# zkonduit/ezkl

Hardware: NVIDIA H100
Metric: prove_time_s (lower is better)
Workload: dtype u32 limbs (254-bit Montgomery integers mod BN254 r/p)

## Files before the change

### ezkl_b200/csrc/capi.cu

```cuda
#include <atomic>
#include <cerrno>
#include <condition_variable>
#include <cstdlib>
#include <cstring>
#include <deque>
#include <functional>
#include <mutex>
#include <string>
#include <thread>
#include <unordered_map>
#include <vector>

#include "../../include/ezkl_b200.h"
#include "msm.cuh"
#include "ntt.cuh"
#include "poly.cuh"
#include "quotient.cuh"

namespace b200 {

static Config g_cfg;
const Config& config() { return g_cfg; }
int sm_count() {
    static std::atomic<int> cache[64];
    int dev = 0;
    if (cudaGetDevice(&dev) != cudaSuccess || dev < 0 || dev >= 64) return 132;
    int v = cache[dev].load(std::memory_order_relaxed);
    if (v == 0) {
        if (cudaDeviceGetAttribute(&v, cudaDevAttrMultiProcessorCount, dev) != cudaSuccess || v <= 0) v = 132;
        cache[dev].store(v, std::memory_order_relaxed);
    }
    return v;
}
static int env_int(const char* name, int dflt) { const char* e = getenv(name); return e ? atoi(e) : dflt; }
static int read_config() {
    Config c;
    if (const char* e = getenv("B200_MSM_TABLE_MB")) {
        char* end = nullptr;
        errno = 0;
        const unsigned long long mb = strtoull(e, &end, 10);
        B200_CHECK(*e >= '0' && *e <= '9' && *end == '\0' && errno == 0 && mb >= 1 && mb < ((unsigned long long)1 << 40), -1,
                   "b200_init: B200_MSM_TABLE_MB = '%s' is not a positive whole number of MiB", e);
        c.msm_table_budget = (size_t)mb << 20;
    }
    if (const char* e = getenv("B200_WS_BUDGET_MB")) c.ws_budget_call = (size_t)atol(e) << 20;
    if (const char* e = getenv("B200_WS_TOTAL_MB")) c.ws_budget_total = (size_t)atol(e) << 20;
    c.msm_reduce_m = env_int("B200_MSM_REDUCE_M", 0);
    c.msm_reduce_threads = env_int("B200_MSM_REDUCE_THREADS", 0);
    c.shard_min_logn = env_int("B200_SHARD_MIN_LOGN", 22);
    g_cfg = c;
    return 0;
}

static constexpr int MAX_DEV = 8;
struct DeviceState { int id = -1; NttContext ntt; };
static DeviceState g_devs[MAX_DEV];
static std::atomic<int> g_ndev{0};
static std::atomic<bool> g_inited{false};
static std::atomic<int> g_active{0};
static std::atomic<uint64_t> g_epoch{1};
static std::mutex g_mu;

struct BaseSet {
    size_t n = 0; int c = 0, W = 0, s = 1, L = 0;
    MsmTable* t[MAX_DEV] = {};
};
static std::unordered_map<uint64_t, BaseSet*> g_tables;
static uint64_t g_next_handle = 1;

struct Ctx {
    int slot = 0, dev = 0;
    cudaStream_t stream = nullptr;
    MsmWorkspace msm_ws;
    PolyWorkspace poly_ws;
    QuotientWorkspace quot_ws;
    StagingRing ring;
    DevBuf stage_a, stage_b, stage_c, small;
    uint8_t* bounce[2] = {nullptr, nullptr};
    cudaEvent_t bounce_ev[2] = {nullptr, nullptr};
    cudaEvent_t last_ev = nullptr;
    cudaStream_t last_stream = nullptr;
    bool has_last = false;
    void release() {
        cudaSetDevice(dev);
        DevBuf* bufs[] = {&msm_ws.counts, &msm_ws.offs, &msm_ws.ents, &msm_ws.subs, &msm_ws.sums, &msm_ws.misc, &poly_ws.scratch, &quot_ws.prog,
                          &stage_a, &stage_b, &stage_c, &small};
        for (DevBuf* b : bufs) b->release();
        ring.release(); poly_ws.ring.release(); quot_ws.ring.release();
        for (int i = 0; i < 2; ++i) { if (bounce[i]) cudaFreeHost(bounce[i]); if (bounce_ev[i]) cudaEventDestroy(bounce_ev[i]); bounce[i] = nullptr; bounce_ev[i] = nullptr; }
        if (last_ev) cudaEventDestroy(last_ev);
        if (stream) cudaStreamDestroy(stream);
        last_ev = nullptr; stream = nullptr;
    }
};
static std::vector<Ctx*> g_ctxs;
static std::atomic<int> g_nctx{0};

struct TlCtx {
    Ctx* c[MAX_DEV] = {};
    uint64_t epoch = 0;
    ~TlCtx() {
        if (epoch != g_epoch.load() || !g_inited.load()) return;
        std::lock_guard<std::mutex> lk(g_mu);
        if (epoch != g_epoch.load()) return;
        int cur = 0; cudaGetDevice(&cur);
        for (int s = 0; s < MAX_DEV; ++s) if (c[s]) {
            for (size_t i = 0; i < g_ctxs.size(); ++i) if (g_ctxs[i] == c[s]) { g_ctxs.erase(g_ctxs.begin() + i); break; }
            c[s]->release(); delete c[s]; g_nctx--;
        }
        cudaSetDevice(cur);
    }
};
static thread_local TlCtx tl;

struct CallGuard {
    bool ok;
    CallGuard() { g_active++; ok = g_inited.load(); if (!ok) set_error("b200: not initialised (call b200_init first)"); }
    ~CallGuard() { g_active--; }
};

static int get_ctx(Ctx** out, int slot = 0) {
    if (!g_inited.load()) { set_error("b200: not initialised (call b200_init first)"); return -3; }
    const uint64_t ep = g_epoch.load();
    if (tl.epoch != ep) { for (int s = 0; s < MAX_DEV; ++s) tl.c[s] = nullptr; tl.epoch = ep; }
    B200_CHECK(slot >= 0 && slot < g_ndev.load(), -1, "b200: device slot %d out of range", slot);
    if (!tl.c[slot]) {
        Ctx* c = new Ctx();
        c->slot = slot; c->dev = g_devs[slot].id;
        int cur = 0; cudaGetDevice(&cur);
        cudaError_t e = cudaSetDevice(c->dev);
        if (e == cudaSuccess) e = cudaStreamCreateWithFlags(&c->stream, cudaStreamNonBlocking);
        if (e == cudaSuccess) e = cudaEventCreateWithFlags(&c->last_ev, cudaEventDisableTiming);
        if (g_ndev.load() > 1) cudaSetDevice(cur);
        if (e != cudaSuccess) { set_error("b200: context creation on device %d failed: %s", c->dev, cudaGetErrorString(e)); delete c; return -2; }
        std::lock_guard<std::mutex> lk(g_mu);
        g_ctxs.push_back(c); g_nctx++;
        tl.c[slot] = c;
    }
    *out = tl.c[slot];
    return 0;
}
static int slot_of(const void* dptr) {
    const int nd = g_ndev.load();
    if (nd <= 1 || !dptr) return 0;
    cudaPointerAttributes at;
    if (cudaPointerGetAttributes(&at, dptr) != cudaSuccess) { cudaGetLastError(); return 0; }
    for (int s = 0; s < nd; ++s) if (g_devs[s].id == at.device) return s;
    return 0;
}
struct DevGuard {
    int prev = -1;
    explicit DevGuard(const Ctx* c) { if (g_ndev.load() > 1) { cudaGetDevice(&prev); if (prev != c->dev) cudaSetDevice(c->dev); else prev = -1; } }
    ~DevGuard() { if (prev >= 0) cudaSetDevice(prev); }
};
struct StreamScope {
    Ctx* c; cudaStream_t st;
    StreamScope(Ctx* c_, void* user) : c(c_), st(user ? (cudaStream_t)user : c_->stream) {
        if (c->has_last && c->last_stream != st) cudaStreamWaitEvent(st, c->last_ev, 0);
    }
    ~StreamScope() { if (cudaEventRecord(c->last_ev, st) == cudaSuccess) { c->last_stream = st; c->has_last = true; } else cudaGetLastError(); }
};
#define B200_ENTER(c, dptr)                                                \
    CallGuard _cg; if (!_cg.ok) return -3;                                 \
    Ctx* c; if (int _rc = get_ctx(&c, slot_of(dptr))) return _rc;          \
    DevGuard _dg(c)

static size_t call_budget() {
    if (g_cfg.ws_budget_call) return g_cfg.ws_budget_call;
// ... 1090 lines not shown
```

### ezkl_b200/csrc/debug.cu

```cuda
#include "../../include/ezkl_b200.h"
#include "msm.cuh"
#include "ntt.cuh"

namespace b200 {
template <class Tag>
__global__ void k_dbg_field(int op, const Fp<Tag>* a, const Fp<Tag>* b, Fp<Tag>* o, size_t n) {
    size_t i = (size_t)blockIdx.x * blockDim.x + threadIdx.x;
    if (i >= n) return;
    Fp<Tag> x = fp_load(a + i), y = fp_load(b + i), r;
    if (op == 0) r = x + y; else if (op == 1) r = x - y; else if (op == 2) r = x * y; else if (op == 3) r = fp_inv(x); else r = fp_from_mont(x);
    fp_store(o + i, r);
}
__global__ void k_dbg_g1(int op, const G1Affine* a, const G1Affine* b, G1Affine* o, size_t n) {
    size_t i = (size_t)blockIdx.x * blockDim.x + threadIdx.x;
    if (i >= n) return;
    G1Affine p = a[i], q = b[i];
    G1Xyzz r;
    if (op == 0) r = g1_add_mixed(g1_to_xyzz(p), q);
    else if (op == 1) r = g1_dbl(g1_to_xyzz(p));
    else if (op == 2) r = g1_mul_small(g1_to_xyzz(p), q.x.l[0]);
    else if (op == 3) r = g1_add(g1_to_xyzz(p), g1_dbl_affine(q));
    else r = g1_add_mixed(g1_to_xyzz(p), g1_neg(p));
    o[i] = g1_to_affine(r);
}
__global__ void k_dbg_digits(const Fr* s, int c, int W, int32_t* out, size_t n) {
    size_t i = (size_t)blockIdx.x * blockDim.x + threadIdx.x;
    if (i >= n) return;
    Fr v = fp_from_mont(fp_load(s + i));
    uint32_t carry = 0;
    for (int w = 0; w < W; ++w) out[i * W + w] = msm_next_digit(v.l, c, &carry);
}
template <int VARIANT>
__global__ void __launch_bounds__(256) k_bench_mul(Fq* out, int iters) {
    const uint32_t t = blockIdx.x * blockDim.x + threadIdx.x;
    Fq x = fp_one<FqTag>(), y = fp_one<FqTag>();
    x.l[0] ^= t; y.l[1] ^= (t * 2654435761u);
    if (VARIANT == 0) {
#pragma unroll 1
        for (int i = 0; i < iters; ++i) x = x * y;
    } else if (VARIANT == 1) {
        Fq z = y + y;
#pragma unroll 1
        for (int i = 0; i < iters; i += 2) { x = x * y; z = z * y; }
        x = x + z;
    } else if (VARIANT == 2) {
#pragma unroll 1
        for (int i = 0; i < iters; ++i) { Fq r; fp_mul_portable<FqTag>(r.l, x.l, y.l); x = r; }
    } else if (VARIANT == 3) {
        G1Affine g; g.x = x; g.y = y;
        G1Xyzz acc = g1_dbl_affine(g);
#pragma unroll 1
        for (int i = 0; i < iters; ++i) { acc = g1_add_mixed(acc, g); g.x.l[0] += 1; }
        x = acc.x + acc.y + acc.zz + acc.zzz;
    } else {
#pragma unroll 1
        for (int i = 0; i < iters; ++i) { x = x + y; y = y - x; }
    }
    fp_store(out + t, x);
}
template <int V>
__global__ void __launch_bounds__(256) k_bench_pipe(uint64_t* out, int iters) {
    const uint32_t t = blockIdx.x * blockDim.x + threadIdx.x;
    uint32_t a = t * 2654435761u + 12345u, b = t ^ 0x9e3779b9u;
    if (V == 0) {
        uint64_t c0 = t, c1 = t + 1, c2 = t + 2, c3 = t + 3, c4 = t + 4, c5 = t + 5, c6 = t + 6, c7 = t + 7;
#pragma unroll 1
        for (int i = 0; i < iters; ++i) {
            asm volatile("mad.wide.u32 %0, %8, %9, %0;\n\tmad.wide.u32 %1, %8, %9, %1;\n\tmad.wide.u32 %2, %8, %9, %2;\n\tmad.wide.u32 %3, %8, %9, %3;\n\t"
                         "mad.wide.u32 %4, %8, %9, %4;\n\tmad.wide.u32 %5, %8, %9, %5;\n\tmad.wide.u32 %6, %8, %9, %6;\n\tmad.wide.u32 %7, %8, %9, %7;"
                         : "+l"(c0), "+l"(c1), "+l"(c2), "+l"(c3), "+l"(c4), "+l"(c5), "+l"(c6), "+l"(c7) : "r"(a), "r"(b));
        }
        out[t] = c0 ^ c1 ^ c2 ^ c3 ^ c4 ^ c5 ^ c6 ^ c7;
    } else if (V == 1) {
        uint32_t e0 = t, e1 = 1, e2 = 2, e3 = 3, e4 = 4, e5 = 5, e6 = 6, e7 = 7, o0 = 8, o1 = 9, o2 = 10, o3 = 11, o4 = 12, o5 = 13, o6 = 14, o7 = 15;
#pragma unroll 1
        for (int i = 0; i < iters; ++i) {
            asm volatile("mad.lo.cc.u32 %0, %16, %17, %0;\n\tmadc.hi.cc.u32 %1, %16, %17, %1;\n\tmadc.lo.cc.u32 %2, %16, %17, %2;\n\tmadc.hi.cc.u32 %3, %16, %17, %3;\n\t"
                         "madc.lo.cc.u32 %4, %16, %17, %4;\n\tmadc.hi.cc.u32 %5, %16, %17, %5;\n\tmadc.lo.cc.u32 %6, %16, %17, %6;\n\tmadc.hi.u32 %7, %16, %17, %7;\n\t"
                         "mad.lo.cc.u32 %8, %16, %17, %8;\n\tmadc.hi.cc.u32 %9, %16, %17, %9;\n\tmadc.lo.cc.u32 %10, %16, %17, %10;\n\tmadc.hi.cc.u32 %11, %16, %17, %11;\n\t"
                         "madc.lo.cc.u32 %12, %16, %17, %12;\n\tmadc.hi.cc.u32 %13, %16, %17, %13;\n\tmadc.lo.cc.u32 %14, %16, %17, %14;\n\tmadc.hi.u32 %15, %16, %17, %15;"
                         : "+r"(e0), "+r"(e1), "+r"(e2), "+r"(e3), "+r"(e4), "+r"(e5), "+r"(e6), "+r"(e7), "+r"(o0), "+r"(o1), "+r"(o2), "+r"(o3), "+r"(o4), "+r"(o5), "+r"(o6), "+r"(o7)
                         : "r"(a), "r"(b));
        }
        out[t] = (uint64_t)(e0 ^ e1 ^ e2 ^ e3 ^ e4 ^ e5 ^ e6 ^ e7) << 32 | (o0 ^ o1 ^ o2 ^ o3 ^ o4 ^ o5 ^ o6 ^ o7);
    } else if (V == 2) {
        uint32_t c0 = t, c1 = 1, c2 = 2, c3 = 3, c4 = 4, c5 = 5, c6 = 6, c7 = 7;
#pragma unroll 1
        for (int i = 0; i < iters; ++i) {
            asm volatile("mad.lo.u32 %0, %8, %9, %0;\n\tmad.lo.u32 %1, %8, %9, %1;\n\tmad.lo.u32 %2, %8, %9, %2;\n\tmad.lo.u32 %3, %8, %9, %3;\n\t"
                         "mad.lo.u32 %4, %8, %9, %4;\n\tmad.lo.u32 %5, %8, %9, %5;\n\tmad.lo.u32 %6, %8, %9, %6;\n\tmad.lo.u32 %7, %8, %9, %7;"
                         : "+r"(c0), "+r"(c1), "+r"(c2), "+r"(c3), "+r"(c4), "+r"(c5), "+r"(c6), "+r"(c7) : "r"(a), "r"(b));
        }
        out[t] = c0 ^ c1 ^ c2 ^ c3 ^ c4 ^ c5 ^ c6 ^ c7;
    } else {
        double x = (double)a, y = 1.0 + 1e-9 * (double)(b & 1023), c0 = t, c1 = 1, c2 = 2, c3 = 3, c4 = 4, c5 = 5, c6 = 6, c7 = 7;
#pragma unroll 1
        for (int i = 0; i < iters; ++i) {
            c0 = fma(x, y, c0); c1 = fma(x, y, c1); c2 = fma(x, y, c2); c3 = fma(x, y, c3); c4 = fma(x, y, c4); c5 = fma(x, y, c5); c6 = fma(x, y, c6); c7 = fma(x, y, c7);
        }
        out[t] = (uint64_t)(c0 + c1 + c2 + c3 + c4 + c5 + c6 + c7);
    }
}
}
using namespace b200;

#pragma GCC visibility push(default)
extern "C" {
// ... 16 lines not shown
    B200_CUDA(cudaGetLastError());
    B200_CUDA(cudaMemcpy(out, dout, 64 * n, cudaMemcpyDeviceToHost));
    cudaFree(da); cudaFree(db); cudaFree(dout);
    return 0;
}
int b200_debug_digits(const b200_fr* s, size_t n, int c, int32_t* out ) {
    const int W = (255 + c - 1) / c;
    void *ds, *dout;
    B200_CUDA(cudaMalloc(&ds, 32 * n)); B200_CUDA(cudaMalloc(&dout, 4 * n * W));
    B200_CUDA(cudaMemcpy(ds, s, 32 * n, cudaMemcpyHostToDevice));
    k_dbg_digits<<<div_up(n, 128), 128>>>((const Fr*)ds, c, W, (int32_t*)dout, n);
    B200_CUDA(cudaGetLastError());
    B200_CUDA(cudaMemcpy(out, dout, 4 * n * W, cudaMemcpyDeviceToHost));
    cudaFree(ds); cudaFree(dout);
    return 0;
}
int b200_debug_bench(int variant, int iters, int blocks, int threads, float* ms) {
    Fq* d; B200_CUDA(cudaMalloc(&d, sizeof(Fq) * (size_t)blocks * threads));
    cudaEvent_t e0, e1; cudaEventCreate(&e0); cudaEventCreate(&e1);
    for (int rep = 0; rep < 2; ++rep) {
        cudaEventRecord(e0);
        switch (variant) {
            case 0: k_bench_mul<0><<<blocks, threads>>>(d, iters); break;
            case 1: k_bench_mul<1><<<blocks, threads>>>(d, iters); break;
            case 2: k_bench_mul<2><<<blocks, threads>>>(d, iters); break;
            case 3: k_bench_mul<3><<<blocks, threads>>>(d, iters); break;
            default: k_bench_mul<4><<<blocks, threads>>>(d, iters); break;
        }
        cudaEventRecord(e1);
        B200_CUDA(cudaEventSynchronize(e1));
    }
    B200_CUDA(cudaEventElapsedTime(ms, e0, e1));
    cudaFree(d); cudaEventDestroy(e0); cudaEventDestroy(e1);
    return 0;
}
int b200_debug_bench_pipe(int variant, int iters, int blocks, int threads, float* ms) {
    uint64_t* d; B200_CUDA(cudaMalloc(&d, 8 * (size_t)blocks * threads));
    cudaEvent_t e0, e1; cudaEventCreate(&e0); cudaEventCreate(&e1);
    for (int rep = 0; rep < 2; ++rep) {
        cudaEventRecord(e0);
        switch (variant) {
            case 0: k_bench_pipe<0><<<blocks, threads>>>(d, iters); break;
            case 1: k_bench_pipe<1><<<blocks, threads>>>(d, iters); break;
            case 2: k_bench_pipe<2><<<blocks, threads>>>(d, iters); break;
            default: k_bench_pipe<3><<<blocks, threads>>>(d, iters); break;
        }
        cudaEventRecord(e1);
        B200_CUDA(cudaEventSynchronize(e1));
    }
    B200_CUDA(cudaEventElapsedTime(ms, e0, e1));
    cudaFree(d); cudaEventDestroy(e0); cudaEventDestroy(e1);
    return 0;
}
int b200_debug_digits_host(const b200_fr* s_canonical, size_t n, int c, int32_t* out) {
    const int W = (255 + c - 1) / c;
    for (size_t i = 0; i < n; ++i) {
        uint32_t v[8]; memcpy(v, &s_canonical[i], 32);
        uint32_t carry = 0;
        for (int w = 0; w < W; ++w) out[i * W + w] = msm_next_digit(v, c, &carry);
    }
    return 0;
}
int b200_debug_digit_slots_host(const b200_fr* s_canonical, size_t n, int c, int wpl, int32_t* out) {
    const int W = (255 + c - 1) / c;
    for (size_t i = 0; i < n; ++i) {
        uint32_t v[8]; memcpy(v, &s_canonical[i], 32);
        uint32_t carry = 0;
        MsmWindowSlot slot;
        for (int w = 0; w < W; ++w) {
            const int32_t d = msm_next_digit(v, c, &carry);
            int32_t* o = out + ((size_t)i * W + w) * 4;
            o[0] = (int32_t)slot.level; o[1] = slot.r;
            o[2] = d ? (int32_t)(slot.set_off + (uint32_t)(d < 0 ? -d : d) - 1u) : -1;
            o[3] = d < 0 ? -1 : (d > 0 ? 1 : 0);
            slot.next(c, wpl);
        }
    }
    return 0;
}
int b200_debug_msm_pick_levels(size_t n, int c, size_t max_table_bytes, int* s, int* L) {
    msm_pick_levels(n, c, max_table_bytes, s, L);
    return 0;
}
int b200_debug_ntt_plan_host(uint32_t log_n, int batch, int sm_count, int64_t* out ) {
    if (log_n < 1 || log_n > 28 || batch < 1 || batch > 65535 || sm_count < 1) return -1;
    int npass, logm[3];
    ntt_choose_passes(log_n, &npass, logm);
    for (int i = 0; i < npass; ++i) {
        const NttPassShape sh = ntt_pass_shape(npass, logm, i);
        const NttPassGeom g = ntt_pass_geometry((uint32_t)logm[i], sh.inner_cnt, sh.lines, batch, sm_count);
        int64_t* o = out + 7 * i;
        o[0] = g.kernel; o[1] = logm[i]; o[2] = g.log_g; o[3] = g.threads; o[4] = (int64_t)g.smem; o[5] = (int64_t)g.grid_x;
        o[6] = i == npass - 1 ? 0 : (g.kernel == 2 && ntt_full_table(log_n, npass) ? 1 : 2);
    }
    return npass;
}
int b200_debug_host_g1_op(int op, const b200_g1_affine* a, const b200_g1_affine* b, b200_g1_affine* out, size_t n) {
    for (size_t i = 0; i < n; ++i) {
        G1Affine p, q; memcpy(&p, &a[i], 64); memcpy(&q, &b[i], 64);
        G1Xyzz r;
        if (op == 0) r = g1_add_mixed(g1_to_xyzz(p), q);
        else if (op == 1) r = g1_dbl(g1_to_xyzz(p));
        else if (op == 2) r = g1_mul_small(g1_to_xyzz(p), q.x.l[0]);
        else if (op == 3) r = g1_add(g1_to_xyzz(p), g1_dbl_affine(q));
        else r = g1_add_mixed(g1_to_xyzz(p), g1_neg(p));
        G1Affine o = g1_to_affine(r); memcpy(&out[i], &o, 64);
    }
    return 0;
}
int b200_debug_host_field_op(int field, int op, const b200_fr* a, const b200_fr* b, b200_fr* out, size_t n) {
    for (size_t i = 0; i < n; ++i) {
        if (field == 0) { Fr x, y, r; memcpy(&x, &a[i], 32); memcpy(&y, &b[i], 32);
            if (op == 0) r = x + y; else if (op == 1) r = x - y; else if (op == 2) r = x * y; else if (op == 3) r = fp_inv(x); else r = fp_from_mont(x);
            memcpy(&out[i], &r, 32);
        } else { Fq x, y, r; memcpy(&x, &a[i], 32); memcpy(&y, &b[i], 32);
            if (op == 0) r = x + y; else if (op == 1) r = x - y; else if (op == 2) r = x * y; else if (op == 3) r = fp_inv(x); else r = fp_from_mont(x);
            memcpy(&out[i], &r, 32);
        }
    }
    return 0;
}
}
#pragma GCC visibility pop
```

### ezkl_b200/csrc/msm.cu

```cuda
#include "msm.cuh"
#include "ec_coop.cuh"

namespace b200 {

static constexpr int HEAVY_CHUNKS = 32;
static constexpr int REDUCE_M_MAX = 32;
static constexpr int TREE_THREADS = 256;

int msm_default_window(size_t n) {
    int k = 0;
    while (((size_t)1 << (k + 1)) <= n) ++k;
    int c = k <= 10 ? 8 : (k <= 13 ? k - 2 : (k <= 17 ? k - 1 : (k <= 19 ? 17 : (k <= 21 ? 18 : 20))));
    if (c < 4) c = 4;
    if (c > 22) c = 22;
    return c;
}

__global__ void __launch_bounds__(128) k_table_next_level(const G1Affine* __restrict__ prev, G1Affine* __restrict__ next, size_t n, int c) {
    size_t i = (size_t)blockIdx.x * blockDim.x + threadIdx.x;
    if (i >= n) return;
    G1Affine p = prev[i];
    G1Xyzz a = g1_dbl_affine(p);
#pragma unroll 1
    for (int j = 1; j < c; ++j) a = g1_dbl(a);
    next[i] = g1_to_affine(a);
}

int msm_table_alloc(MsmTable* t, size_t n, int c, size_t max_table_bytes) {
    B200_CHECK(n > 0, -1, "msm_table_build: empty base vector");
    if (c <= 0) c = msm_default_window(n);
    int W = (255 + c - 1) / c, s = 1, L = W;
    msm_pick_levels(n, c, max_table_bytes, &s, &L);
    B200_CHECK((size_t)L * n < ((size_t)1 << 31), -1, "msm_table_build: L*n = %zu exceeds the 31-bit entry index", (size_t)L * n);
    t->n = n; t->c = c; t->W = W; t->s = s; t->L = L;
    B200_CUDA(cudaGetDevice(&t->device));
    const cudaError_t e = cudaMalloc(&t->d_table, t->bytes());
    if (e != cudaSuccess) {
        cudaGetLastError();
        t->d_table = nullptr;
        set_error("msm_table_build: %zu MiB table (%d levels of %zu points): %s", t->bytes() >> 20, L, n, cudaGetErrorString(e));
        return -2;
    }
    return 0;
}

int msm_table_build(MsmTable* t, const G1Affine* d_bases, cudaStream_t st) {
    const size_t n = t->n;
    if (d_bases) B200_CUDA(cudaMemcpyAsync(t->d_table, d_bases, sizeof(G1Affine) * n, cudaMemcpyDeviceToDevice, st));
    for (int j = 1; j < t->L; ++j) {
        k_table_next_level<<<div_up(n, 128), 128, 0, st>>>(t->d_table + (size_t)(j - 1) * n, t->d_table + (size_t)j * n, n, t->c * t->s); count_launch();
    }
    B200_CUDA(cudaGetLastError());
    return 0;
}
void msm_table_free(MsmTable* t) {
    if (t->d_table) cudaFree(t->d_table);
    t->d_table = nullptr;
}

template <bool SCATTER, bool SUBWIN>
__global__ void __launch_bounds__(256) k_digits(const Fr* __restrict__ scalars, size_t stride, uint32_t n, uint32_t table_n, uint32_t base_off, int c, int W,
                                                 uint32_t nbuckets, uint32_t* __restrict__ counters ,
                                                 const uint32_t* __restrict__ offs , uint32_t* __restrict__ ents, size_t ent_stride,
                                                 const uint32_t* __restrict__ skew, int wpl) {
    const uint32_t col = blockIdx.y;
    const bool aggregate = !SCATTER || skew[col] != 0;
    const Fr* sc = scalars + (size_t)col * stride;
    uint32_t* cnt = counters + (size_t)col * nbuckets;
    const uint32_t* off = SCATTER ? offs + (size_t)col * (nbuckets + 1) : nullptr;
    uint32_t* ent = SCATTER ? ents + (size_t)col * ent_stride : nullptr;
    const unsigned lane = threadIdx.x & 31;
    const uint32_t n_up = (n + 31u) & ~31u;
    for (uint32_t i = blockIdx.x * blockDim.x + threadIdx.x; i < n_up; i += gridDim.x * blockDim.x) {
        const bool valid = i < n;
        Fr s = fp_zero<FrTag>();
        if (valid) s = fp_from_mont(fp_load(sc + i));
        uint32_t carry = 0;
        MsmWindowSlot slot;
#pragma unroll 1
        for (int w = 0; w < W; ++w) {
            int32_t d = msm_next_digit(s.l, c, &carry);
            const uint32_t j = SUBWIN ? slot.level : (uint32_t)w;
            const bool nz = d != 0;
            const unsigned act = __ballot_sync(0xffffffffu, nz);
            if (nz && !aggregate) {
                const uint32_t bucket = (SUBWIN ? slot.set_off : 0u) + (uint32_t)(d < 0 ? -d : d) - 1u;
                ent[off[bucket] + atomicAdd(&cnt[bucket], 1u)] = (j * table_n + base_off + i) | (d < 0 ? 0x80000000u : 0u);
            } else if (nz) {
                const uint32_t bucket = (SUBWIN ? slot.set_off : 0u) + (uint32_t)(d < 0 ? -d : d) - 1u;
                const unsigned peers = __match_any_sync(act, bucket);
                const int leader = __ffs(peers) - 1;
                uint32_t base = 0;
                if ((int)lane == leader) base = atomicAdd(&cnt[bucket], (uint32_t)__popc(peers));
                if (SCATTER) {
                    base = __shfl_sync(peers, base, leader);
                    const uint32_t rank = __popc(peers & ((1u << lane) - 1u));
                    ent[off[bucket] + base + rank] = (j * table_n + base_off + i) | (d < 0 ? 0x80000000u : 0u);
                }
            }
            if (SUBWIN) slot.next(c, wpl);
        }
    }
}

__global__ void __launch_bounds__(1024) k_scan_buckets(const uint32_t* __restrict__ counts, uint32_t* __restrict__ offs, uint32_t* __restrict__ chunk_offs,
                                                        uint32_t nbuckets, uint32_t cap, uint32_t* __restrict__ skew ) {
    __shared__ uint32_t sh_max;
    if (threadIdx.x == 0) sh_max = 0;
    __syncthreads();
    const uint32_t col = blockIdx.x;
    const uint32_t lc = 31u - (uint32_t)__clz(cap);
    const uint32_t* cnt = counts + (size_t)col * nbuckets;
    uint32_t* off = offs + (size_t)col * (nbuckets + 1);
    uint32_t* coff = chunk_offs + (size_t)col * (nbuckets + 1);
    const uint32_t ipt = (nbuckets + blockDim.x - 1) / blockDim.x;
    const uint32_t lo = threadIdx.x * ipt, hi = min(lo + ipt, nbuckets);
    uint32_t s = 0, cs = 0;
    uint32_t mx = 0;
    const bool vec = (ipt & 3u) == 0 && lo + ipt <= nbuckets;
    if (vec) {
        const uint4* c4 = reinterpret_cast<const uint4*>(cnt + lo);
#pragma unroll 4
        for (uint32_t q = 0; q < (ipt >> 2); ++q) {
            const uint4 v = c4[q];
            s += v.x + v.y + v.z + v.w;
            cs += ((v.x + cap - 1) >> lc) + ((v.y + cap - 1) >> lc) + ((v.z + cap - 1) >> lc) + ((v.w + cap - 1) >> lc);
            mx = max(max(mx, v.x), max(max(v.y, v.z), v.w));
        }
    } else {
        for (uint32_t b = lo; b < hi; ++b) { uint32_t v = cnt[b]; s += v; cs += ((v + cap - 1) >> lc); mx = max(mx, v); }
    }
    if (mx) atomicMax(&sh_max, mx);
    uint32_t tot, ctot;
    uint32_t ex = block_exclusive_scan(s, &tot);
    uint32_t cex = block_exclusive_scan(cs, &ctot);
    if (vec) {
        const uint4* c4 = reinterpret_cast<const uint4*>(cnt + lo);
#pragma unroll 4
        for (uint32_t q = 0; q < (ipt >> 2); ++q) {
            const uint4 v = c4[q];
            const uint32_t b = lo + 4 * q;
            off[b] = ex; coff[b] = cex; ex += v.x; cex += ((v.x + cap - 1) >> lc);
            off[b + 1] = ex; coff[b + 1] = cex; ex += v.y; cex += ((v.y + cap - 1) >> lc);
            off[b + 2] = ex; coff[b + 2] = cex; ex += v.z; cex += ((v.z + cap - 1) >> lc);
            off[b + 3] = ex; coff[b + 3] = cex; ex += v.w; cex += ((v.w + cap - 1) >> lc);
        }
    } else {
        for (uint32_t b = lo; b < hi; ++b) { uint32_t v = cnt[b]; off[b] = ex; coff[b] = cex; ex += v; cex += ((v + cap - 1) >> lc); }
    }
    if (threadIdx.x == 0) {
        off[nbuckets] = tot; coff[nbuckets] = ctot;
        skew[col] = sh_max > 16u * (tot / nbuckets + 1u) ? 1u : 0u;
    }
}

__global__ void __launch_bounds__(256) k_fill_chunks(const uint32_t* __restrict__ offs, const uint32_t* __restrict__ chunk_offs, uint32_t nbuckets, uint32_t cap,
                                                      uint32_t* __restrict__ chunk_start, uint32_t* __restrict__ chunk_len, size_t chunk_stride,
                                                      uint32_t* __restrict__ len_hist , uint32_t* __restrict__ heavy , uint32_t heavy_stride) {
    extern __shared__ uint32_t sh_hist[];
    const uint32_t col = blockIdx.y;
    for (uint32_t j = threadIdx.x; j <= cap; j += blockDim.x) sh_hist[j] = 0;
    __syncthreads();
    const uint32_t* off = offs + (size_t)col * (nbuckets + 1);
    const uint32_t* coff = chunk_offs + (size_t)col * (nbuckets + 1);
    uint32_t* cs = chunk_start + (size_t)col * chunk_stride;
    uint32_t* cl = chunk_len + (size_t)col * chunk_stride;
    const uint32_t b = blockIdx.x * blockDim.x + threadIdx.x;
    if (b < nbuckets) {
        const uint32_t start = off[b], size = off[b + 1] - start, c0 = coff[b], nch = coff[b + 1] - c0;
        for (uint32_t j = 0; j < nch; ++j) {
            const uint32_t len = min(cap, size - j * cap);
            cs[c0 + j] = start + j * cap;
            cl[c0 + j] = len;
            if (j + 1 == nch) atomicAdd(&sh_hist[len], 1u);
        }
        if (nch > 1) atomicAdd(&sh_hist[cap], nch - 1);
        if (nch > (uint32_t)HEAVY_CHUNKS) {
            uint32_t* hv = heavy + (size_t)col * heavy_stride;
            uint32_t slot = atomicAdd(&hv[0], 1u);
            if (slot + 1 < heavy_stride) hv[1 + slot] = b;
        }
    }
    __syncthreads();
    uint32_t* gh = len_hist + (size_t)col * (cap + 1);
    for (uint32_t j = threadIdx.x; j <= cap; j += blockDim.x) if (sh_hist[j]) atomicAdd(&gh[j], sh_hist[j]);
// ... 166 lines not shown
    acc = block_sum_coop(acc, sh);
    if (threadIdx.x == 0) out[col] = acc;
}

__global__ void __launch_bounds__(32) k_subwindow_fold(const G1Xyzz* __restrict__ set_sums , int s, int c, uint32_t batch, G1Xyzz* __restrict__ out) {
    const uint32_t col = blockIdx.x * blockDim.x + threadIdx.x;
    if (col >= batch) return;
    const G1Xyzz* rs = set_sums + (size_t)col * s;
    G1Xyzz acc = rs[s - 1];
#pragma unroll 1
    for (int r = s - 2; r >= 0; --r) {
#pragma unroll 1
        for (int k = 0; k < c; ++k) acc = g1_dbl(acc);
        acc = g1_add(acc, rs[r]);
    }
    out[col] = acc;
}

__global__ void __launch_bounds__(128) k_g1_generate(uint64_t seed, size_t n, G1Affine* __restrict__ out) {
    const size_t i = (size_t)blockIdx.x * blockDim.x + threadIdx.x;
    if (i >= n) return;
    uint32_t s[8];
    uint64_t z = seed + 0x9e3779b97f4a7c15ull * (uint64_t)(i + 1);
#pragma unroll
    for (int w = 0; w < 4; ++w) {
        z += 0x9e3779b97f4a7c15ull;
        uint64_t x = z; x = (x ^ (x >> 30)) * 0xbf58476d1ce4e5b9ull; x = (x ^ (x >> 27)) * 0x94d049bb133111ebull; x ^= x >> 31;
        s[2 * w] = (uint32_t)x; s[2 * w + 1] = (uint32_t)(x >> 32);
    }
    s[7] &= 0x0fffffffu;
    G1Affine g; g.x = fp_one<FqTag>(); g.y = fp_one<FqTag>() + fp_one<FqTag>();
    G1Xyzz acc = g1_xyzz_identity();
#pragma unroll 1
    for (int b = 251; b >= 0; --b) {
        acc = g1_dbl(acc);
        if ((s[b >> 5] >> (b & 31)) & 1) acc = g1_add_mixed(acc, g);
    }
    out[i] = g1_to_affine(acc);
}
int g1_generate_run(uint64_t seed, size_t n, G1Affine* d_out, cudaStream_t st) {
    if (n == 0) return 0;
    k_g1_generate<<<div_up(n, 128), 128, 0, st>>>(seed, n, d_out); count_launch();
    B200_CUDA(cudaGetLastError());
    return 0;
}

__global__ void __launch_bounds__(128) k_g1_fixed_base_mul(const Fr* __restrict__ scalars, size_t n, G1Affine base, G1Affine* __restrict__ out) {
    const size_t i = (size_t)blockIdx.x * blockDim.x + threadIdx.x;
    if (i >= n) return;
    const Fr s = fp_from_mont(fp_load(scalars + i));
    G1Xyzz acc = g1_xyzz_identity();
#pragma unroll 1
    for (int b = 253; b >= 0; --b) {
        acc = g1_dbl(acc);
        if ((s.l[b >> 5] >> (b & 31)) & 1) acc = g1_add_mixed(acc, base);
    }
    out[i] = g1_to_affine(acc);
}
int g1_fixed_base_mul_run(const Fr* d_scalars, size_t n, const G1Affine& base, G1Affine* d_out, cudaStream_t st) {
    if (n == 0) return 0;
    k_g1_fixed_base_mul<<<div_up(n, 128), 128, 0, st>>>(d_scalars, n, base, d_out); count_launch();
    B200_CUDA(cudaGetLastError());
    return 0;
}

int g1_sum_run(const G1Xyzz* d_points, size_t groups, size_t count, G1Xyzz* d_out, cudaStream_t st) {
    if (groups == 0) return 0;
    B200_CHECK(groups <= 0x7fffffffu && count <= 0xffffffffu, -1, "g1_sum: sizes out of range");
    k_final_coop<<<(unsigned)groups, TREE_THREADS, 0, st>>>(d_points, (uint32_t)count, d_out); count_launch();
    B200_CUDA(cudaGetLastError());
    return 0;
}

static uint32_t pick_cap(size_t total_entries) {
    size_t target = total_entries / ((size_t)sm_count() * 512 * 4);
    uint32_t cap = 16;
    while (cap < 512 && cap < target) cap <<= 1;
    return cap;
}

size_t msm_workspace_per_column(const MsmTable& t, size_t n) {
    const size_t nb = (size_t)t.s << (t.c - 1), ents = n * t.W;
    const size_t chunk_stride = nb + ents / 16 + 1;
    return ents * 4 + chunk_stride * (12 + sizeof(G1Xyzz)) + nb * (sizeof(G1Xyzz) + 24) + 65536 * (size_t)t.s;
}

int msm_run(const MsmTable& t, const Fr* d_scalars, size_t n, size_t stride, int batch, G1Xyzz* d_out, MsmWorkspace& ws, cudaStream_t st, size_t base_off) {
    B200_CHECK(base_off + n <= t.n, -1, "msm: pairs [%zu, %zu) but only %zu bases registered", base_off, base_off + n, t.n);
    B200_CHECK(batch > 0 && batch <= 65535, -1, "msm: batch %d out of range", batch);
    if (n == 0) {
        B200_CUDA(cudaMemsetAsync(d_out, 0, sizeof(G1Xyzz) * batch, st));
        return 0;
    }
    const int c = t.c, W = t.W, s = t.s;
    B200_CHECK((size_t)batch * s <= 65535, -1, "msm: batch %d x %d bucket sets out of range", batch, s);
    const uint32_t half = 1u << (c - 1), nb = half * (uint32_t)s;
    const int vcols = batch * s;
    const size_t ent_stride = (size_t)n * W;
    B200_CHECK(ent_stride < ((size_t)1 << 32), -1, "msm: n*W too large");
    const Config& cfg = config();
    const uint32_t cap = pick_cap(ent_stride * batch);
    const size_t chunk_stride = (size_t)nb + ent_stride / cap + 1;
    const uint32_t heavy_stride = (uint32_t)(ent_stride / ((size_t)cap * HEAVY_CHUNKS)) + 2;
    const size_t all_buckets = (size_t)batch * nb;
    uint32_t reduce_m = REDUCE_M_MAX, reduce_threads = TREE_THREADS;
    if (all_buckets <= ((size_t)1 << 15)) { reduce_m = 4; reduce_threads = 128; }
    else if (all_buckets <= ((size_t)1 << 18)) { reduce_m = 8; reduce_threads = 128; }
    else if (all_buckets <= ((size_t)5 << 17)) { reduce_m = 16; reduce_threads = 256; }
    else if (all_buckets < ((size_t)37 << 15)) { reduce_m = 32; reduce_threads = 128; }
    while (reduce_m > 1 && reduce_m > half) reduce_m >>= 1;
    if (cfg.msm_reduce_m >= 1 && cfg.msm_reduce_m <= 4096) reduce_m = (uint32_t)cfg.msm_reduce_m;
    if (cfg.msm_reduce_threads == 32 || cfg.msm_reduce_threads == 64 || cfg.msm_reduce_threads == 128 || cfg.msm_reduce_threads == 256) reduce_threads = (uint32_t)cfg.msm_reduce_threads;
    const uint32_t nparts = div_up(div_up(half, reduce_m), reduce_threads);
    uint32_t final_threads = 32;
    while (final_threads < (uint32_t)TREE_THREADS && final_threads < nparts) final_threads <<= 1;

    const size_t n_hist = (size_t)batch * nb, n_len = (size_t)batch * (cap + 1), n_heavy = (size_t)batch * heavy_stride;
    const size_t counts_words = 2 * n_hist + 2 * n_len + n_heavy;
    if (ws.counts.ensure(counts_words * 4)) return -2;
    uint32_t* hist = ws.counts.as<uint32_t>();
    uint32_t* cursor = hist + n_hist;
    uint32_t* len_hist = cursor + n_hist;
    uint32_t* len_cursor = len_hist + n_len;
    uint32_t* heavy = len_cursor + n_len;
    const size_t n_off = (size_t)batch * (nb + 1);
    if (ws.offs.ensure((2 * n_off + n_len + (size_t)batch) * 4)) return -2;
    uint32_t* offs = ws.offs.as<uint32_t>();
    uint32_t* chunk_offs = offs + n_off;
    uint32_t* len_offs = chunk_offs + n_off;
    uint32_t* skew = len_offs + n_len;
    if (ws.ents.ensure((size_t)batch * ent_stride * 4)) return -2;
    uint32_t* ents = ws.ents.as<uint32_t>();
    if (ws.subs.ensure((size_t)batch * chunk_stride * 4 * 3)) return -2;
    uint32_t* chunk_start = ws.subs.as<uint32_t>();
    uint32_t* chunk_len = chunk_start + (size_t)batch * chunk_stride;
    uint32_t* order = chunk_len + (size_t)batch * chunk_stride;
    const size_t n_set = s > 1 ? (size_t)vcols : 0;
    if (ws.sums.ensure(sizeof(G1Xyzz) * ((size_t)batch * chunk_stride + (size_t)batch * nb + (size_t)vcols * nparts + n_set))) return -2;
    G1Xyzz* chunk_sums = ws.sums.as<G1Xyzz>();
    G1Xyzz* bucket_sums = chunk_sums + (size_t)batch * chunk_stride;
    G1Xyzz* partials = bucket_sums + (size_t)batch * nb;
    G1Xyzz* reduced = s > 1 ? partials + (size_t)vcols * nparts : d_out;

    ProfScope ps_total(PROF_MSM_TOTAL, st);
    B200_CUDA(cudaMemsetAsync(hist, 0, counts_words * 4, st));
    if (prof_enabled()) prof_mark(PROF_MSM_RECODE, st, true);
    const unsigned sms = (unsigned)sm_count();
    const unsigned dig_blocks = min(div_up(n, 256), sms * 8u);
    dim3 gd(dig_blocks, batch);
    if (s == 1) k_digits<false, false><<<gd, 256, 0, st>>>(d_scalars, stride, (uint32_t)n, (uint32_t)t.n, (uint32_t)base_off, c, W, nb, hist, nullptr, nullptr, 0, nullptr, 1);
    else k_digits<false, true><<<gd, 256, 0, st>>>(d_scalars, stride, (uint32_t)n, (uint32_t)t.n, (uint32_t)base_off, c, W, nb, hist, nullptr, nullptr, 0, nullptr, s);
    count_launch();
    {
        ProfScope ps(PROF_MSM_SCAN, st);
        k_scan_buckets<<<batch, 1024, 0, st>>>(hist, offs, chunk_offs, nb, cap, skew); count_launch();
    }
    if (s == 1) k_digits<true, false><<<gd, 256, 0, st>>>(d_scalars, stride, (uint32_t)n, (uint32_t)t.n, (uint32_t)base_off, c, W, nb, cursor, offs, ents, ent_stride, skew, 1);
    else k_digits<true, true><<<gd, 256, 0, st>>>(d_scalars, stride, (uint32_t)n, (uint32_t)t.n, (uint32_t)base_off, c, W, nb, cursor, offs, ents, ent_stride, skew, s);
    count_launch();
    k_fill_chunks<<<dim3(div_up(nb, 256), batch), 256, (cap + 1) * 4, st>>>(offs, chunk_offs, nb, cap, chunk_start, chunk_len, chunk_stride, len_hist, heavy, heavy_stride); count_launch();
    k_len_offsets<<<batch, 32, 0, st>>>(len_hist, len_offs, cap); count_launch();
    const unsigned ch_blocks = min(div_up(chunk_stride, 256), sms * 8u);
    k_order_chunks<<<dim3(ch_blocks, batch), 256, 0, st>>>(chunk_len, chunk_stride, chunk_offs, nb, len_offs, len_cursor, cap, order); count_launch();
    if (prof_enabled()) prof_mark(PROF_MSM_RECODE, st, false);
    const unsigned acc_blocks = min(div_up(chunk_stride, 128), sms * 16u);
    {
        ProfScope ps(PROF_MSM_ACCUMULATE, st);
        k_accumulate<<<dim3(acc_blocks, batch), 128, 0, st>>>(t.d_table, ents, ent_stride, chunk_start, chunk_len, order, chunk_stride, chunk_offs, nb, chunk_sums); count_launch();
    }
    ProfScope ps_tail(PROF_MSM_TAIL, st);
    k_combine<<<dim3(div_up(nb, 128), batch), 128, 0, st>>>(chunk_offs, nb, chunk_sums, chunk_stride, bucket_sums); count_launch();
    k_combine_heavy<<<dim3(32, batch), TREE_THREADS, 0, st>>>(heavy, heavy_stride, chunk_offs, nb, chunk_sums, chunk_stride, bucket_sums); count_launch();
    {
        ProfScope ps(PROF_MSM_REDUCE, st);
        k_reduce<1><<<dim3(nparts, vcols), reduce_threads, 0, st>>>(bucket_sums, half, partials, nparts, reduce_m); count_launch();
        k_final<<<vcols, final_threads, 0, st>>>(partials, nparts, reduced); count_launch();
    }
    if (s > 1) {
        ProfScope ps(PROF_MSM_FOLD, st);
        k_subwindow_fold<<<div_up((size_t)batch, 32), 32, 0, st>>>(reduced, s, c, (uint32_t)batch, d_out); count_launch();
    }
    B200_CUDA(cudaGetLastError());
    return 0;
}

}
```

### ezkl_b200/csrc/msm.cuh

```cuda
#pragma once
#include "common.cuh"
#include "ec.cuh"

namespace b200 {

struct MsmTable {
    G1Affine* d_table = nullptr;
    size_t n = 0;
    int c = 0;
    int W = 0;
    int s = 1;
    int L = 0;
    int device = 0;
    size_t bytes() const { return sizeof(G1Affine) * n * (size_t)L; }
};

struct MsmWorkspace {
    DevBuf counts, offs, ents, subs, sums, misc;
};

int msm_default_window(size_t n);
inline void msm_pick_levels(size_t n, int c, size_t max_table_bytes, int* s, int* L) {
    const int W = (255 + c - 1) / c;
    const size_t level_bytes = sizeof(G1Affine) * n;
    for (int k = 1; k <= W; ++k) {
        const int l = (W + k - 1) / k;
        if (k == W || (size_t)l * level_bytes <= max_table_bytes) { *s = k; *L = l; return; }
    }
}
int msm_table_alloc(MsmTable* t, size_t n, int c, size_t max_table_bytes);
int msm_table_build(MsmTable* t, const G1Affine* d_bases, cudaStream_t st);
void msm_table_free(MsmTable* t);
int msm_run(const MsmTable& t, const Fr* d_scalars, size_t n, size_t stride, int batch, G1Xyzz* d_out,
            MsmWorkspace& ws, cudaStream_t st, size_t base_off = 0);
int g1_fixed_base_mul_run(const Fr* d_scalars, size_t n, const G1Affine& base, G1Affine* d_out, cudaStream_t st);
int g1_fft_run(const G1Affine* d_in, uint32_t log_n, const Fr& omega, const Fr* scale, G1Affine* d_out, DevBuf& scratch, cudaStream_t st);
int g1_generate_run(uint64_t seed, size_t n, G1Affine* d_out, cudaStream_t st);
int g1_sum_run(const G1Xyzz* d_points, size_t groups, size_t count, G1Xyzz* d_out, cudaStream_t st);
size_t msm_workspace_per_column(const MsmTable& t, size_t n);

HD int32_t msm_next_digit(uint32_t s[8], int c, uint32_t* carry) {
    uint32_t v = (s[0] & ((1u << c) - 1u)) + *carry;
#pragma unroll
    for (int j = 0; j < 7; ++j) s[j] = (s[j] >> c) | (s[j + 1] << (32 - c));
    s[7] >>= c;
    if (v > (1u << (c - 1))) { *carry = 1; return (int32_t)v - (int32_t)(1u << c); }
    *carry = 0;
    return (int32_t)v;
}

struct MsmWindowSlot {
    uint32_t level = 0, set_off = 0;
    int r = 0;
    HD void next(int c, int wpl) {
        set_off += 1u << (c - 1);
        if (++r == wpl) { r = 0; set_off = 0; ++level; }
    }
};

}
```

Baseline: 0.08932.

## Use tiled shared-memory bucket histograms for MSM digit recoding

Replaces the global-atomic count and scatter passes of MSM scalar recoding with a tiled scheme. Each block builds a per-tile bucket histogram in shared memory, a prefix kernel turns the per-tile counts into offsets, and a second tiled pass scatters entries using shared-memory cursors. The goal is to remove contended global atomics and keep scatter writes local within each tile. The cost is extra workspace for tile counts, an extra kernel launch, and 1024-thread blocks with up to 128KB of shared memory, which limits occupancy. Debug shims and a base-offset test entry point are added as well.

```diff
diff --git a/ezkl_b200/csrc/capi.cu b/ezkl_b200/csrc/capi.cu
--- a/ezkl_b200/csrc/capi.cu
+++ b/ezkl_b200/csrc/capi.cu
@@ -83,7 +83,7 @@
     bool has_last = false;
     void release() {
         cudaSetDevice(dev);
-        DevBuf* bufs[] = {&msm_ws.counts, &msm_ws.offs, &msm_ws.ents, &msm_ws.subs, &msm_ws.sums, &msm_ws.misc, &poly_ws.scratch, &quot_ws.prog,
+        DevBuf* bufs[] = {&msm_ws.counts, &msm_ws.offs, &msm_ws.ents, &msm_ws.subs, &msm_ws.sums, &msm_ws.misc, &msm_ws.tile_counts, &poly_ws.scratch, &quot_ws.prog,
                           &stage_a, &stage_b, &stage_c, &small};
         for (DevBuf* b : bufs) b->release();
         ring.release(); poly_ws.ring.release(); quot_ws.ring.release();
diff --git a/ezkl_b200/csrc/debug.cu b/ezkl_b200/csrc/debug.cu
--- a/ezkl_b200/csrc/debug.cu
+++ b/ezkl_b200/csrc/debug.cu
@@ -23,6 +23,19 @@
     else r = g1_add_mixed(g1_to_xyzz(p), g1_neg(p));
     o[i] = g1_to_affine(r);
 }
+__global__ void k_dbg_xyzz_to_affine(const G1Xyzz* p, G1Affine* o, size_t n) {
+    size_t i = (size_t)blockIdx.x * blockDim.x + threadIdx.x;
+    if (i < n) o[i] = g1_to_affine(p[i]);
+}
+static Config g_dbg_cfg;
+const Config& config() { return g_dbg_cfg; }
+int sm_count() {
+    int dev = 0, v = 0;
+    if (cudaGetDevice(&dev) != cudaSuccess || cudaDeviceGetAttribute(&v, cudaDevAttrMultiProcessorCount, dev) != cudaSuccess || v <= 0) return 132;
+    return v;
+}
+bool prof_enabled() { return false; }
+void prof_mark(int, cudaStream_t, bool) {}
 __global__ void k_dbg_digits(const Fr* s, int c, int W, int32_t* out, size_t n) {
     size_t i = (size_t)blockIdx.x * blockDim.x + threadIdx.x;
     if (i >= n) return;
@@ -205,6 +218,40 @@
     msm_pick_levels(n, c, max_table_bytes, s, L);
     return 0;
 }
+int b200_debug_msm_recode_plan(size_t n, int batch, uint32_t nbuckets, int W, int sm_count, uint32_t* out ) {
+    const MsmRecodePlan p = msm_pick_recode(n, batch, nbuckets, W, sm_count);
+    out[0] = p.tile; out[1] = p.tiles;
+    return 0;
+}
+int b200_debug_msm_base_off(const b200_fr* scalars, size_t n, int batch, const b200_g1_affine* bases, size_t table_n, int c,
+                            size_t max_table_bytes, size_t base_off, b200_g1_affine* out) {
+    if (n == 0 || batch < 1 || batch > 4096 || base_off + n > table_n || c < 4 || c > 22) return -1;
+    MsmTable t;
+    MsmWorkspace ws;
+    void *d_sc = nullptr, *d_xyzz = nullptr, *d_aff = nullptr;
+    auto run = [&]() -> int {
+        if (int rc = msm_table_alloc(&t, table_n, c, max_table_bytes ? max_table_bytes : ~(size_t)0)) return rc;
+        B200_CUDA(cudaMemcpy(t.d_table, bases, sizeof(G1Affine) * table_n, cudaMemcpyHostToDevice));
+        if (int rc = msm_table_build(&t, nullptr, 0)) return rc;
+        B200_CUDA(cudaMalloc(&d_sc, sizeof(Fr) * n * batch));
+        B200_CUDA(cudaMalloc(&d_xyzz, sizeof(G1Xyzz) * batch));
+        B200_CUDA(cudaMalloc(&d_aff, sizeof(G1Affine) * batch));
+        B200_CUDA(cudaMemcpy(d_sc, scalars, sizeof(Fr) * n * batch, cudaMemcpyHostToDevice));
+        if (int rc = msm_run(t, (const Fr*)d_sc, n, n, batch, (G1Xyzz*)d_xyzz, ws, 0, base_off)) return rc;
+        k_dbg_xyzz_to_affine<<<div_up(batch, 32), 32>>>((const G1Xyzz*)d_xyzz, (G1Affine*)d_aff, (size_t)batch);
+        B200_CUDA(cudaGetLastError());
+        B200_CUDA(cudaMemcpy(out, d_aff, sizeof(G1Affine) * batch, cudaMemcpyDeviceToHost));
+        return 0;
+    };
+    const int rc = run();
+    DevBuf* bufs[] = {&ws.counts, &ws.offs, &ws.ents, &ws.subs, &ws.sums, &ws.misc, &ws.tile_counts};
+    for (DevBuf* b : bufs) b->release();
+    msm_table_free(&t);
+    if (d_sc) cudaFree(d_sc);
+    if (d_xyzz) cudaFree(d_xyzz);
+    if (d_aff) cudaFree(d_aff);
+    return rc;
+}
 int b200_debug_ntt_plan_host(uint32_t log_n, int batch, int sm_count, int64_t* out ) {
     if (log_n < 1 || log_n > 28 || batch < 1 || batch > 65535 || sm_count < 1) return -1;
     int npass, logm[3];
diff --git a/ezkl_b200/csrc/msm.cu b/ezkl_b200/csrc/msm.cu
--- a/ezkl_b200/csrc/msm.cu
+++ b/ezkl_b200/csrc/msm.cu
@@ -101,6 +101,63 @@
             if (SUBWIN) slot.next(c, wpl);
         }
     }
+}
+
+template <bool SCATTER, bool SUBWIN>
+__global__ void __launch_bounds__(MSM_TILE_THREADS, 1) k_digits_tile(const Fr* __restrict__ scalars, size_t stride, uint32_t n, uint32_t table_n, uint32_t base_off,
+                                                                     int c, int W, uint32_t nbuckets, uint32_t tile, uint32_t* __restrict__ tile_counts ,
+                                                                     const uint32_t* __restrict__ offs , uint32_t* __restrict__ ents, size_t ent_stride, int wpl) {
+    extern __shared__ uint32_t sh_cnt[];
+    const uint32_t col = blockIdx.y;
+    const Fr* sc = scalars + (size_t)col * stride;
+    uint32_t* tc = tile_counts + ((size_t)col * gridDim.x + blockIdx.x) * nbuckets;
+    if (SCATTER) {
+        const uint32_t* off = offs + (size_t)col * (nbuckets + 1);
+        for (uint32_t b = threadIdx.x; b < nbuckets; b += blockDim.x) sh_cnt[b] = off[b] + tc[b];
+    } else {
+        for (uint32_t b = threadIdx.x; b < nbuckets; b += blockDim.x) sh_cnt[b] = 0;
+    }
+    __syncthreads();
+    uint32_t* ent = SCATTER ? ents + (size_t)col * ent_stride : nullptr;
+    const uint32_t lo = blockIdx.x * tile, hi = min(lo + tile, n);
+    for (uint32_t i = lo + threadIdx.x; i < hi; i += blockDim.x) {
+        Fr s = fp_from_mont(fp_load(sc + i));
+        uint32_t carry = 0;
+        MsmWindowSlot slot;
+#pragma unroll 1
+        for (int w = 0; w < W; ++w) {
+            const int32_t d = msm_next_digit(s.l, c, &carry);
+            if (d != 0) {
+                const uint32_t bucket = (SUBWIN ? slot.set_off : 0u) + (uint32_t)(d < 0 ? -d : d) - 1u;
+                const uint32_t pos = atomicAdd(&sh_cnt[bucket], 1u);
+                if (SCATTER) ent[pos] = ((SUBWIN ? slot.level : (uint32_t)w) * table_n + base_off + i) | (d < 0 ? 0x80000000u : 0u);
+            }
+            if (SUBWIN) slot.next(c, wpl);
+        }
+    }
+    if (!SCATTER) {
+        __syncthreads();
+        for (uint32_t b = threadIdx.x; b < nbuckets; b += blockDim.x) tc[b] = sh_cnt[b];
+    }
+}
+
+__global__ void __launch_bounds__(256) k_tile_prefix(uint32_t* __restrict__ tile_counts, uint32_t tiles, uint32_t nbuckets, uint32_t* __restrict__ hist) {
+    const uint32_t col = blockIdx.y;
+    const uint32_t b = blockIdx.x * blockDim.x + threadIdx.x;
+    if (b >= nbuckets) return;
+    uint32_t* tc = tile_counts + (size_t)col * tiles * nbuckets + b;
+    uint32_t acc = 0;
+    for (uint32_t t0 = 0; t0 < tiles; t0 += 8) {
+        uint32_t v[8];
+#pragma unroll
+        for (int j = 0; j < 8; ++j) v[j] = t0 + j < tiles ? tc[(size_t)(t0 + j) * nbuckets] : 0u;
+#pragma unroll
+        for (int j = 0; j < 8; ++j) {
+            if (t0 + j < tiles) tc[(size_t)(t0 + j) * nbuckets] = acc;
+            acc += v[j];
+        }
+    }
+    hist[(size_t)col * nbuckets + b] = acc;
 }
 
 __global__ void __launch_bounds__(1024) k_scan_buckets(const uint32_t* __restrict__ counts, uint32_t* __restrict__ offs, uint32_t* __restrict__ chunk_offs,
@@ -433,7 +490,8 @@
 size_t msm_workspace_per_column(const MsmTable& t, size_t n) {
     const size_t nb = (size_t)t.s << (t.c - 1), ents = n * t.W;
     const size_t chunk_stride = nb + ents / 16 + 1;
-    return ents * 4 + chunk_stride * (12 + sizeof(G1Xyzz)) + nb * (sizeof(G1Xyzz) + 24) + 65536 * (size_t)t.s;
+    const size_t tile_counts = nb <= MSM_TILE_MAX_BUCKETS ? (ents + nb) * 4 : 0;
+    return ents * 4 + chunk_stride * (12 + sizeof(G1Xyzz)) + nb * (sizeof(G1Xyzz) + 24) + 65536 * (size_t)t.s + tile_counts;
 }
 
 int msm_run(const MsmTable& t, const Fr* d_scalars, size_t n, size_t stride, int batch, G1Xyzz* d_out, MsmWorkspace& ws, cudaStream_t st, size_t base_off) {
@@ -466,6 +524,8 @@
     uint32_t final_threads = 32;
     while (final_threads < (uint32_t)TREE_THREADS && final_threads < nparts) final_threads <<= 1;
 
+    const unsigned sms = (unsigned)sm_count();
+    const MsmRecodePlan rp = msm_pick_recode(n, batch, nb, W, (int)sms);
     const size_t n_hist = (size_t)batch * nb, n_len = (size_t)batch * (cap + 1), n_heavy = (size_t)batch * heavy_stride;
     const size_t counts_words = 2 * n_hist + 2 * n_len + n_heavy;
     if (ws.counts.ensure(counts_words * 4)) return -2;
@@ -474,6 +534,19 @@
     uint32_t* len_hist = cursor + n_hist;
     uint32_t* len_cursor = len_hist + n_len;
     uint32_t* heavy = len_cursor + n_len;
+    uint32_t* zero_from = rp.tile ? len_hist : hist;
+    const size_t zero_words = counts_words - (size_t)(zero_from - hist);
+    uint32_t* tile_counts = nullptr;
+    const size_t tile_smem = (size_t)nb * 4;
+    auto* count_k = s == 1 ? k_digits_tile<false, false> : k_digits_tile<false, true>;
+    auto* place_k = s == 1 ? k_digits_tile<true, false> : k_digits_tile<true, true>;
+    if (rp.tile) {
+        if (ws.tile_counts.ensure((size_t)batch * rp.tiles * nb * 4)) return -2;
+        tile_counts = ws.tile_counts.as<uint32_t>();
+        const int smem_limit = (int)(MSM_TILE_MAX_BUCKETS * 4);
+        B200_CUDA(cudaFuncSetAttribute(count_k, cudaFuncAttributeMaxDynamicSharedMemorySize, smem_limit));
+        B200_CUDA(cudaFuncSetAttribute(place_k, cudaFuncAttributeMaxDynamicSharedMemorySize, smem_limit));
+    }
     const size_t n_off = (size_t)batch * (nb + 1);
     if (ws.offs.ensure((2 * n_off + n_len + (size_t)batch) * 4)) return -2;
     uint32_t* offs = ws.offs.as<uint32_t>();
@@ -494,20 +567,30 @@
     G1Xyzz* reduced = s > 1 ? partials + (size_t)vcols * nparts : d_out;
 
     ProfScope ps_total(PROF_MSM_TOTAL, st);
-    B200_CUDA(cudaMemsetAsync(hist, 0, counts_words * 4, st));
+    B200_CUDA(cudaMemsetAsync(zero_from, 0, zero_words * 4, st));
     if (prof_enabled()) prof_mark(PROF_MSM_RECODE, st, true);
-    const unsigned sms = (unsigned)sm_count();
     const unsigned dig_blocks = min(div_up(n, 256), sms * 8u);
-    dim3 gd(dig_blocks, batch);
-    if (s == 1) k_digits<false, false><<<gd, 256, 0, st>>>(d_scalars, stride, (uint32_t)n, (uint32_t)t.n, (uint32_t)base_off, c, W, nb, hist, nullptr, nullptr, 0, nullptr, 1);
-    else k_digits<false, true><<<gd, 256, 0, st>>>(d_scalars, stride, (uint32_t)n, (uint32_t)t.n, (uint32_t)base_off, c, W, nb, hist, nullptr, nullptr, 0, nullptr, s);
-    count_launch();
+    const dim3 gd(dig_blocks, batch), gt(rp.tiles, batch);
+    if (rp.tile) {
+        count_k<<<gt, MSM_TILE_THREADS, tile_smem, st>>>(d_scalars, stride, (uint32_t)n, (uint32_t)t.n, (uint32_t)base_off, c, W, nb, rp.tile, tile_counts, nullptr, nullptr, 0, s);
+        count_launch();
+        k_tile_prefix<<<dim3(div_up(nb, 256), batch), 256, 0, st>>>(tile_counts, rp.tiles, nb, hist); count_launch();
+    } else {
+        if (s == 1) k_digits<false, false><<<gd, 256, 0, st>>>(d_scalars, stride, (uint32_t)n, (uint32_t)t.n, (uint32_t)base_off, c, W, nb, hist, nullptr, nullptr, 0, nullptr, 1);
+        else k_digits<false, true><<<gd, 256, 0, st>>>(d_scalars, stride, (uint32_t)n, (uint32_t)t.n, (uint32_t)base_off, c, W, nb, hist, nullptr, nullptr, 0, nullptr, s);
+        count_launch();
+    }
     {
         ProfScope ps(PROF_MSM_SCAN, st);
         k_scan_buckets<<<batch, 1024, 0, st>>>(hist, offs, chunk_offs, nb, cap, skew); count_launch();
     }
-    if (s == 1) k_digits<true, false><<<gd, 256, 0, st>>>(d_scalars, stride, (uint32_t)n, (uint32_t)t.n, (uint32_t)base_off, c, W, nb, cursor, offs, ents, ent_stride, skew, 1);
-    else k_digits<true, true><<<gd, 256, 0, st>>>(d_scalars, stride, (uint32_t)n, (uint32_t)t.n, (uint32_t)base_off, c, W, nb, cursor, offs, ents, ent_stride, skew, s);
+    if (rp.tile) {
+        place_k<<<gt, MSM_TILE_THREADS, tile_smem, st>>>(d_scalars, stride, (uint32_t)n, (uint32_t)t.n, (uint32_t)base_off, c, W, nb, rp.tile, tile_counts, offs, ents, ent_stride, s);
+    } else if (s == 1) {
+        k_digits<true, false><<<gd, 256, 0, st>>>(d_scalars, stride, (uint32_t)n, (uint32_t)t.n, (uint32_t)base_off, c, W, nb, cursor, offs, ents, ent_stride, skew, 1);
+    } else {
+        k_digits<true, true><<<gd, 256, 0, st>>>(d_scalars, stride, (uint32_t)n, (uint32_t)t.n, (uint32_t)base_off, c, W, nb, cursor, offs, ents, ent_stride, skew, s);
+    }
     count_launch();
     k_fill_chunks<<<dim3(div_up(nb, 256), batch), 256, (cap + 1) * 4, st>>>(offs, chunk_offs, nb, cap, chunk_start, chunk_len, chunk_stride, len_hist, heavy, heavy_stride); count_launch();
     k_len_offsets<<<batch, 32, 0, st>>>(len_hist, len_offs, cap); count_launch();
diff --git a/ezkl_b200/csrc/msm.cuh b/ezkl_b200/csrc/msm.cuh
--- a/ezkl_b200/csrc/msm.cuh
+++ b/ezkl_b200/csrc/msm.cuh
@@ -16,7 +16,7 @@
 };
 
 struct MsmWorkspace {
-    DevBuf counts, offs, ents, subs, sums, misc;
+    DevBuf counts, offs, ents, subs, sums, misc, tile_counts;
 };
 
 int msm_default_window(size_t n);
@@ -27,6 +27,27 @@
         const int l = (W + k - 1) / k;
         if (k == W || (size_t)l * level_bytes <= max_table_bytes) { *s = k; *L = l; return; }
     }
+}
+struct MsmRecodePlan {
+    uint32_t tile = 0, tiles = 0;
+};
+static constexpr uint32_t MSM_TILE_MAX_BUCKETS = 1u << 15;
+static constexpr uint32_t MSM_TILE_THREADS = 1024;
+static constexpr size_t MSM_TILE_L2_BYTES = (size_t)16 << 20;
+inline MsmRecodePlan msm_pick_recode(size_t n, int batch, uint32_t nb, int W, int sms) {
+    MsmRecodePlan p;
+    if (n == 0 || batch < 1 || W < 1 || sms < 1 || nb == 0 || nb > MSM_TILE_MAX_BUCKETS) return p;
+    const size_t ents = n * (size_t)W;
+    size_t tiles = ((size_t)sms * ents * 4 + MSM_TILE_L2_BYTES - 1) / MSM_TILE_L2_BYTES;
+    const size_t fill = ((size_t)sms + batch - 1) / batch;
+    if (tiles < fill) tiles = fill;
+    size_t tile = (n + tiles - 1) / tiles;
+    const size_t min_tile = (nb + W - 1) / W;
+    if (tile < min_tile) tile = min_tile;
+    tile = (tile + MSM_TILE_THREADS - 1) / MSM_TILE_THREADS * MSM_TILE_THREADS;
+    p.tile = (uint32_t)tile;
+    p.tiles = (uint32_t)((n + tile - 1) / tile);
+    return p;
 }
 int msm_table_alloc(MsmTable* t, size_t n, int c, size_t max_table_bytes);
 int msm_table_build(MsmTable* t, const G1Affine* d_bases, cudaStream_t st);
```

After: 0.08533 (median of 6 runs). 1.05x faster.
